# lachlanhurst/balance-robot-mujoco-rl

Measured on AMD Instinct MI355X. Metric: env-steps/sec, higher is better.
Workload: dtype f32; 1 GPU; Env03-v2, 65536 env instances per GPU (65536 total), random policy U(-1,1)^2, auto-reset on, 250 substeps of 2e-5 s per env step; envs_per_gpu=65536, substeps=250, parallelism=env-sharded x1, no collective, lane_grouping=True, streams=1, preroll_steps=300, preroll_stationary=True

## Files before the change

balance_robot_mujoco_rl_amd/csrc/brs_kernels.hip:

```cpp
#include <hip/hip_runtime.h>

#include <cstdio>
#include <cstdlib>
#include <cstring>
#include <string>
#include <vector>

#include "../../include/brs.h"
#if defined(BRS_TIMING)
__device__ unsigned long long brs_dbg[16];
__device__ unsigned long long brs_dbg_wave[4096];
#define BRS_TIMING_LANE_WORDS 153
#endif
#include "brs_state.hpp"

using namespace brs;

namespace {

template <bool BLK> constexpr int lane_words() { return BLK ? LDS_WORDS_ENV03 : LDS_WORDS_ENV01; }

template <bool BLK> __device__ __forceinline__ Store<float> lane_store(float* lds) {
  const int wave = threadIdx.x >> 6, lane = threadIdx.x & 63;
  return Store<float>{lds + wave * (64 * lane_words<BLK>()) + lane, 64};
}

template <int VARIANT> __device__ __forceinline__ Params<float> fold_params(const Params<float>& rt) {
  if constexpr (VARIANT < 0) return rt;
  else {
    constexpr Params<float> c = make_params<float>(VARIANT, 0u, -1, 0, 0, 0.0, 0, 0);
    Params<float> p = c;
    p.seed = rt.seed; p.gid_base = rt.gid_base; p.auto_reset = rt.auto_reset; p.noise = rt.noise;
    p.max_episode_steps = rt.max_episode_steps; p.nsub = rt.nsub;
    return p;
  }
}

constexpr int NBUCKET = 6;
__device__ __forceinline__ int bucket_of(int key, int e) {
  const int k = key & 3;
  if (k == 1) return 0;
  if (k == 2) return 4;
  if (k == 3) return 5;
  return (key & 4) ? ((e & 1) ? 3 : 1) : 2;
}
constexpr int GROUP_WORDS = 16;
template <bool BLK> __device__ __forceinline__ unsigned* group_counters(int* ii, int N) {
  return (unsigned*)(ii + ((size_t)Layout<BLK>::NI + 2) * N);
}

template <bool BLK, int VARIANT>
__device__ __forceinline__ void step_body(const Params<float>& Prt, const int N, double* __restrict__ d, float* __restrict__ f,
                                          int* __restrict__ ii, const float* __restrict__ actions, float* __restrict__ obs,
                                          float* __restrict__ reward, uint8_t* __restrict__ terminated,
                                          uint8_t* __restrict__ truncated, float* __restrict__ terminal_obs) {
  extern __shared__ float brs_lds_dyn[];
  float* lds = brs_lds_dyn;
  const int lane_slot = blockIdx.x * blockDim.x + threadIdx.x;
  if (lane_slot >= N) return;
  const Params<float> P = fold_params<VARIANT>(Prt);
#if defined(BRS_NO_PERM)
  const LaneIndex idx{nullptr, lane_slot};
#else
  const LaneIndex idx{BLK ? ii + (size_t)Layout<BLK>::NI * N : nullptr, lane_slot};
#endif
  Store<float> st = lane_store<BLK>(lds);
#if defined(BRS_TIMING) && defined(__HIP_DEVICE_COMPILE__)
  if ((threadIdx.x & 63) == 0) for (int k = 0; k < 16; k++) brs_tim_slots()[k] = 0;
#endif
  Stream<float> rng;
  float a0, a1;
  {
    const size_t i = idx.get();
    rng.open(P.seed, P.gid_base + (int64_t)i, 0u);
    a0 = actions[2 * i]; a1 = actions[2 * i + 1];
  }
  float o[6], to[6], rew;
  int te, tr, cls = 0;
  env_step_idx<float, BLK, float, LaneIndex>(P, st, rng, d, f, ii, (size_t)N, idx, a0, a1, o, to, rew, te, tr, BLK ? &cls : nullptr);
  const size_t i = idx.get();
  if constexpr (BLK) {
    ((uint8_t*)(ii + ((size_t)Layout<BLK>::NI + 1) * N))[i] = (uint8_t)cls;
    const int b = bucket_of(cls, (int)i);
    unsigned* cnt = group_counters<BLK>(ii, N);
#pragma unroll
    for (int k = 0; k < NBUCKET; k++) {
      const unsigned long long m = __ballot(b == k);
      if (m != 0ull && (threadIdx.x & 63) == (unsigned)(__ffsll((long long)m) - 1)) atomicAdd(&cnt[k], (unsigned)__popcll(m));
    }
  }
#if defined(BRS_TIMING) && defined(__HIP_DEVICE_COMPILE__)
  if ((threadIdx.x & 63) == 0) {
    for (int k = 0; k < 12; k++) atomicAdd(&brs_dbg[k], brs_tim_slots()[k]);
    atomicMax(&brs_dbg[12], brs_tim_slots()[8]);
    atomicMax(&brs_dbg[13], brs_tim_slots()[9]);
    unsigned hw, xcc;
    asm volatile("s_getreg_b32 %0, hwreg(HW_REG_HW_ID)" : "=s"(hw));
    asm volatile("s_getreg_b32 %0, hwreg(HW_REG_XCC_ID)" : "=s"(xcc));
    const unsigned w = (blockIdx.x * blockDim.x + threadIdx.x) >> 6;
    if (w < 1024) {
      brs_dbg_wave[4 * w + 0] = brs_tim_slots()[8]; brs_dbg_wave[4 * w + 1] = brs_tim_slots()[9];
      brs_dbg_wave[4 * w + 2] = hw; brs_dbg_wave[4 * w + 3] = xcc;
    }
  }
#endif
#pragma unroll
  for (int k = 0; k < 6; k++) obs[6 * (size_t)i + k] = o[k];
  if (terminal_obs) {
#pragma unroll
    for (int k = 0; k < 6; k++) terminal_obs[6 * (size_t)i + k] = to[k];
  }
  reward[i] = rew;
  terminated[i] = (uint8_t)te;
  truncated[i] = (uint8_t)tr;
}

#define BRS_STEP_ARGS                                                                                                      \
  const Params<float> Prt, const int N, double *__restrict__ d, float *__restrict__ f, int *__restrict__ ii,              \
      const float *__restrict__ actions, float *__restrict__ obs, float *__restrict__ reward, uint8_t *__restrict__ terminated, \
      uint8_t *__restrict__ truncated, float *__restrict__ terminal_obs
template <bool BLK, int VARIANT> __global__ void __launch_bounds__(256) brs_step_kernel(BRS_STEP_ARGS) {
  step_body<BLK, VARIANT>(Prt, N, d, f, ii, actions, obs, reward, terminated, truncated, terminal_obs);
}
template <int VARIANT> __global__ void __launch_bounds__(64, 2) brs_step_kernel_occ2(BRS_STEP_ARGS) {
  step_body<false, VARIANT>(Prt, N, d, f, ii, actions, obs, reward, terminated, truncated, terminal_obs);
}

template <bool BLK>
__global__ void __launch_bounds__(256) brs_reset_kernel(const Params<float> P, const int N, double* __restrict__ d,
                                                        float* __restrict__ f, int* __restrict__ ii,
                                                        const uint8_t* __restrict__ mask, float* __restrict__ obs) {
  const int i = blockIdx.x * blockDim.x + threadIdx.x;
  if (i >= N) return;
  if (mask && !mask[i]) return;
  EnvState<float, BLK> S;
  load_state<float, BLK>(S, d, f, ii, (size_t)N, (size_t)i);
  Stream<float> rng;
  rng.open(P.seed, P.gid_base + (int64_t)i, S.rng_ctr);
  float o[6];
  Sim<float, BLK>::env_reset(P, S, rng, o);
  S.rng_ctr = rng.ctr;
  store_state<float, BLK>(S, d, f, ii, (size_t)N, (size_t)i);
#pragma unroll
  for (int k = 0; k < 6; k++) obs[6 * (size_t)i + k] = o[k];
}

template <bool BLK>
__global__ void __launch_bounds__(256) brs_physics_kernel(const Params<float> P, const int N, double* __restrict__ d,
                                                          float* __restrict__ f, int* __restrict__ ii,
                                                          const float* __restrict__ ctrl, const int nsub) {
  extern __shared__ float brs_lds_dyn[];
  float* lds = brs_lds_dyn;
  const int i = blockIdx.x * blockDim.x + threadIdx.x;
  if (i >= N) return;
  Store<float> st = lane_store<BLK>(lds);
  physics_mem<float, BLK, float>(P, st, d, f, ii, (size_t)N, (size_t)i, ctrl[2 * (size_t)i], ctrl[2 * (size_t)i + 1], nsub);
}

constexpr int GROUP_THREADS = 256, GROUP_ENVS = 1024;
__global__ void __launch_bounds__(GROUP_THREADS) brs_group_kernel(const int N, const uint8_t* __restrict__ keys, int* __restrict__ perm,
                                                                  unsigned* __restrict__ ctr) {
  constexpr int NV = GROUP_ENVS / 64;
  __shared__ unsigned wcnt[NV][NBUCKET], woff[NBUCKET];
  const int lane = threadIdx.x & 63, w = threadIdx.x >> 6;
  int b[GROUP_ENVS / GROUP_THREADS];
  unsigned long long mine[GROUP_ENVS / GROUP_THREADS];
#pragma unroll
  for (int j = 0; j < GROUP_ENVS / GROUP_THREADS; j++) {
    const int e = blockIdx.x * GROUP_ENVS + j * GROUP_THREADS + threadIdx.x;
    b[j] = e < N ? bucket_of(keys[e], e) : -1;
    mine[j] = 0ull;
#pragma unroll
    for (int k = 0; k < NBUCKET; k++) {
      const unsigned long long m = __ballot(b[j] == k);
      if (lane == 0) wcnt[j * (GROUP_THREADS / 64) + w][k] = (unsigned)__popcll(m);
      mine[j] = b[j] == k ? m : mine[j];
    }
  }
  __syncthreads();
  if (threadIdx.x < NBUCKET) {
    const int k = threadIdx.x;
    unsigned base = 0, tot = 0;
    for (int j = 0; j < k; j++) base += ctr[j];
    for (int v = 0; v < NV; v++) { const unsigned c = wcnt[v][k]; wcnt[v][k] = tot; tot += c; }
    woff[k] = base + (tot ? atomicAdd(&ctr[NBUCKET + k], tot) : 0u);
  }
  __syncthreads();
#pragma unroll
  for (int j = 0; j < GROUP_ENVS / GROUP_THREADS; j++) {
    const int e = blockIdx.x * GROUP_ENVS + j * GROUP_THREADS + threadIdx.x;
    if (b[j] >= 0) perm[woff[b[j]] + wcnt[j * (GROUP_THREADS / 64) + w][b[j]] + (unsigned)__popcll(mine[j] & ((1ull << lane) - 1ull))] = e;
  }
  __syncthreads();
  if (threadIdx.x == 0) {
    __threadfence();
    if (atomicAdd(&ctr[2 * NBUCKET], 1u) == gridDim.x - 1) {
#pragma unroll
      for (int k = 0; k <= 2 * NBUCKET; k++) ctr[k] = 0u;
    }
  }
}

thread_local std::string g_create_error;

}

struct brs_handle {
  Params<float> P;
  int N = 0, device = 0, bt = 64;
  bool blk = false;
  double* d = nullptr;
  float* f = nullptr;
  int* ii = nullptr;
  size_t nd = 0, nf = 0, ni = 0;
  bool folded = false;
  bool occ2 = false;
  bool grouping = false;
  int* perm() const { return ii + ni; }
  uint8_t* keys() const { return (uint8_t*)(ii + ni + (size_t)N); }
  unsigned* counters() const { return (unsigned*)(ii + ni + 2 * (size_t)N); }
  std::string err;
};

namespace {

struct DeviceGuard {
  int prev = -1;
  bool ok = true;
  explicit DeviceGuard(int dev) {
    if (hipGetDevice(&prev) != hipSuccess) prev = -1;
    if (prev != dev) ok = hipSetDevice(dev) == hipSuccess;
  }
  ~DeviceGuard() {
    if (prev >= 0) (void)hipSetDevice(prev);
  }
};

int fail(brs_handle* h, int code, const std::string& msg) {
  if (h) h->err = msg; else g_create_error = msg;
  return code;
}
#define BRS_HIP_TRY(h, expr)                                                                              \
  do {                                                                                                    \
    hipError_t e_ = (expr);                                                                               \
    if (e_ != hipSuccess) return fail(h, BRS_ERR_HIP, std::string(#expr) + ": " + hipGetErrorString(e_)); \
  } while (0)

#if defined(BRS_TIMING)
size_t lds_bytes(const brs_handle* h) { return (size_t)h->bt * BRS_TIMING_LANE_WORDS * sizeof(float) + (size_t)(h->bt / 64) * 128; }
#else
size_t lds_bytes(const brs_handle* h) { return (size_t)h->bt * (h->blk ? LDS_WORDS_ENV03 : LDS_WORDS_ENV01) * sizeof(float); }
#endif
int grid_of(const brs_handle* h) { return (h->N + h->bt - 1) / h->bt; }

template <bool BLK> int upload_state(brs_handle* h, const std::vector<double>& d, const std::vector<float>& f, const std::vector<int>& ii) {
  BRS_HIP_TRY(h, hipMemcpy(h->d, d.data(), d.size() * sizeof(double), hipMemcpyHostToDevice));
  BRS_HIP_TRY(h, hipMemcpy(h->f, f.data(), f.size() * sizeof(float), hipMemcpyHostToDevice));
  BRS_HIP_TRY(h, hipMemcpy(h->ii, ii.data(), ii.size() * sizeof(int), hipMemcpyHostToDevice));
  return BRS_OK;
}
int download_state(brs_handle* h, std::vector<double>& d, std::vector<float>& f, std::vector<int>& ii) {
  d.resize(h->nd); f.resize(h->nf); ii.resize(h->ni);
  BRS_HIP_TRY(h, hipDeviceSynchronize());
  BRS_HIP_TRY(h, hipMemcpy(d.data(), h->d, h->nd * sizeof(double), hipMemcpyDeviceToHost));
  BRS_HIP_TRY(h, hipMemcpy(f.data(), h->f, h->nf * sizeof(float), hipMemcpyDeviceToHost));
  BRS_HIP_TRY(h, hipMemcpy(ii.data(), h->ii, h->ni * sizeof(int), hipMemcpyDeviceToHost));
  return BRS_OK;
}

}

extern "C" {

int brs_sizes(int32_t variant, int32_t* nq, int32_t* nv, int32_t* nobs, int32_t* nact) {
  if (variant < 0 || variant > 5) return BRS_ERR_ARG;
  bool blk = variant == 2 || variant == 3;
  if (nq) *nq = blk ? 16 : 9;
  if (nv) *nv = blk ? 14 : 8;
  if (nobs) *nobs = 6;
  if (nact) *nact = 2;
  return BRS_OK;
}

int brs_create(const brs_config* cfg, brs_handle** out) {
  if (!cfg || !out) return fail(nullptr, BRS_ERR_ARG, "brs_create: null argument");
  *out = nullptr;
  if (cfg->variant < 0 || cfg->variant > 5) return fail(nullptr, BRS_ERR_ARG, "brs_create: unknown variant");
  if (cfg->num_envs <= 0) return fail(nullptr, BRS_ERR_ARG, "brs_create: num_envs must be > 0");
  if ((cfg->flags & BRS_FLAG_NOISE_ON) && (cfg->flags & BRS_FLAG_NOISE_OFF))
    return fail(nullptr, BRS_ERR_ARG, "brs_create: NOISE_ON and NOISE_OFF are exclusive");
  int bt = cfg->block_threads > 0 ? cfg->block_threads : 64;
  if (bt % 64 != 0 || bt > 256) return fail(nullptr, BRS_ERR_ARG, "brs_create: block_threads must be 64, 128, 192 or 256");
  int ndev = 0;
  hipError_t e = hipGetDeviceCount(&ndev);
  if (e != hipSuccess || ndev <= 0)
    return fail(nullptr, BRS_ERR_HIP, std::string("brs_create: no HIP device (") + hipGetErrorString(e) + "); there is no CPU fallback");
  if (cfg->device < 0 || cfg->device >= ndev) return fail(nullptr, BRS_ERR_ARG, "brs_create: device ordinal out of range");
  brs_handle* h = new brs_handle();
  h->N = cfg->num_envs; h->device = cfg->device; h->bt = bt; h->blk = cfg->variant == 2 || cfg->variant == 3;
  int noise = (cfg->flags & BRS_FLAG_NOISE_ON) ? 1 : ((cfg->flags & BRS_FLAG_NOISE_OFF) ? 0 : -1);
  h->P = make_params<float>(cfg->variant, cfg->flags & BRS_FLAG_AUTO_RESET, noise, cfg->max_episode_steps, cfg->substeps,
                            cfg->timestep, cfg->seed, cfg->env_index_base);
  DeviceGuard g(h->device);
  size_t N = (size_t)h->N;
  if (h->blk) { h->nd = Layout<true>::ND * N; h->nf = Layout<true>::NF * N; h->ni = Layout<true>::NI * N; }
  else { h->nd = Layout<false>::ND * N; h->nf = Layout<false>::NF * N; h->ni = Layout<false>::NI * N; }
  auto bail = [&](const std::string& m) { std::string mm = m; brs_destroy(h); return fail(nullptr, BRS_ERR_HIP, mm); };
  if (!g.ok) return bail("brs_create: hipSetDevice failed");
  if (hipMalloc(&h->d, (h->nd + 7 * N) * sizeof(double)) != hipSuccess) return bail("brs_create: hipMalloc(fp64 state) failed");
  if (hipMalloc(&h->f, h->nf * sizeof(float)) != hipSuccess) return bail("brs_create: hipMalloc(fp32 state) failed");
  if (hipMalloc(&h->ii, (h->ni + 2 * N + GROUP_WORDS) * sizeof(int)) != hipSuccess) return bail("brs_create: hipMalloc(int state) failed");
  std::vector<double> d(h->nd);
  std::vector<float> f(h->nf);
  std::vector<int> ii(h->ni);
  int rc;
  if (h->blk) { hostconv::init_state<true>(d.data(), f.data(), ii.data(), N, cfg->seed, cfg->env_index_base); rc = upload_state<true>(h, d, f, ii); }
  else { hostconv::init_state<false>(d.data(), f.data(), ii.data(), N, cfg->seed, cfg->env_index_base); rc = upload_state<false>(h, d, f, ii); }
  if (rc != BRS_OK) return bail("brs_create: initial upload failed: " + h->err);
  {
    std::vector<int> id(2 * N, 0);
    for (size_t k = 0; k < N; k++) id[k] = (int)k;
    if (hipMemcpy(h->perm(), id.data(), 2 * N * sizeof(int), hipMemcpyHostToDevice) != hipSuccess) return bail("brs_create: lane map init failed");
    if (hipMemset(h->counters(), 0, GROUP_WORDS * sizeof(int)) != hipSuccess) return bail("brs_create: counter init failed");
    h->grouping = h->blk && !(cfg->flags & BRS_FLAG_NO_LANE_GROUPING);
    h->folded = !(cfg->timestep > 0 && cfg->timestep != 2e-5) && !std::getenv("BRS_NO_FOLD");
    h->occ2 = !h->blk && std::getenv("BRS_ENV01_OCC1") == nullptr;
  }
  size_t lb = lds_bytes(h);
  hipError_t ea = hipSuccess;
  auto want = [&](const void* fn) { if (ea == hipSuccess) ea = hipFuncSetAttribute(fn, hipFuncAttributeMaxDynamicSharedMemorySize, (int)lb); };
  if (h->blk) {
    want((const void*)brs_step_kernel<true, -1>); want((const void*)brs_step_kernel<true, ENV03_V1>);
    want((const void*)brs_step_kernel<true, ENV03_V2>); want((const void*)brs_physics_kernel<true>);
  } else {
    want((const void*)brs_step_kernel<false, -1>); want((const void*)brs_step_kernel<false, ENV01_V1>);
    want((const void*)brs_step_kernel<false, ENV01_V2>); want((const void*)brs_step_kernel<false, ENV01_V3>);
    want((const void*)brs_step_kernel<false, ENV02_V1>); want((const void*)brs_physics_kernel<false>);
    want((const void*)brs_step_kernel_occ2<-1>); want((const void*)brs_step_kernel_occ2<ENV01_V1>);
    want((const void*)brs_step_kernel_occ2<ENV01_V2>); want((const void*)brs_step_kernel_occ2<ENV01_V3>);
    want((const void*)brs_step_kernel_occ2<ENV02_V1>);
  }
  if (ea != hipSuccess) return bail(std::string("brs_create: hipFuncSetAttribute: ") + hipGetErrorString(ea));
  *out = h;
  return BRS_OK;
}

int brs_destroy(brs_handle* h) {
  if (!h) return BRS_ERR_STATE;
  {
    DeviceGuard g(h->device);
    if (h->d) (void)hipFree(h->d);
    if (h->f) (void)hipFree(h->f);
    if (h->ii) (void)hipFree(h->ii);
  }
  delete h;
  return BRS_OK;
}

const char* brs_last_error(const brs_handle* h) { return h ? h->err.c_str() : g_create_error.c_str(); }

int brs_reset(brs_handle* h, const uint8_t* mask_dev, float* obs_dev, void* stream) {
  if (!h) return BRS_ERR_STATE;
  if (!obs_dev) return fail(h, BRS_ERR_ARG, "brs_reset: obs_dev is null");
  DeviceGuard g(h->device);
  hipStream_t s = (hipStream_t)stream;
  if (h->blk) hipLaunchKernelGGL(brs_reset_kernel<true>, dim3(grid_of(h)), dim3(h->bt), 0, s, h->P, h->N, h->d, h->f, h->ii, mask_dev, obs_dev);
  else hipLaunchKernelGGL(brs_reset_kernel<false>, dim3(grid_of(h)), dim3(h->bt), 0, s, h->P, h->N, h->d, h->f, h->ii, mask_dev, obs_dev);
  BRS_HIP_TRY(h, hipGetLastError());
  return BRS_OK;
}

int brs_step(brs_handle* h, const float* actions_dev, float* obs_dev, float* reward_dev, uint8_t* terminated_dev,
             uint8_t* truncated_dev, float* terminal_obs_dev, void* stream) {
  if (!h) return BRS_ERR_STATE;
  if (!actions_dev || !obs_dev || !reward_dev || !terminated_dev || !truncated_dev)
    return fail(h, BRS_ERR_ARG, "brs_step: null buffer");
  DeviceGuard g(h->device);
  hipStream_t s = (hipStream_t)stream;
  size_t lb = lds_bytes(h);
  const dim3 grid(grid_of(h)), block(h->bt);
#define BRS_LAUNCH_STEP(BLK_, VAR_)                                                                                          \
  hipLaunchKernelGGL((brs_step_kernel<BLK_, VAR_>), grid, block, lb, s, h->P, h->N, h->d, h->f, h->ii, actions_dev, obs_dev, \
                     reward_dev, terminated_dev, truncated_dev, terminal_obs_dev)
#define BRS_LAUNCH_OCC2(VAR_)                                                                                              \
  hipLaunchKernelGGL((brs_step_kernel_occ2<VAR_>), grid, block, lb, s, h->P, h->N, h->d, h->f, h->ii, actions_dev, obs_dev, \
                     reward_dev, terminated_dev, truncated_dev, terminal_obs_dev)
  if (!h->blk && h->occ2 && h->bt == 64) {
    switch (h->folded ? h->P.variant : -1) {
      case ENV01_V1: BRS_LAUNCH_OCC2(ENV01_V1); break;
      case ENV01_V2: BRS_LAUNCH_OCC2(ENV01_V2); break;
      case ENV01_V3: BRS_LAUNCH_OCC2(ENV01_V3); break;
      case ENV02_V1: BRS_LAUNCH_OCC2(ENV02_V1); break;
      default: BRS_LAUNCH_OCC2(-1);
    }
  } else
  switch (h->folded ? h->P.variant : -1) {
    case ENV01_V1: BRS_LAUNCH_STEP(false, ENV01_V1); break;
    case ENV01_V2: BRS_LAUNCH_STEP(false, ENV01_V2); break;
    case ENV01_V3: BRS_LAUNCH_STEP(false, ENV01_V3); break;
    case ENV02_V1: BRS_LAUNCH_STEP(false, ENV02_V1); break;
    case ENV03_V1: BRS_LAUNCH_STEP(true, ENV03_V1); break;
    case ENV03_V2: BRS_LAUNCH_STEP(true, ENV03_V2); break;
    default:
      if (h->blk) BRS_LAUNCH_STEP(true, -1); else BRS_LAUNCH_STEP(false, -1);
  }
#undef BRS_LAUNCH_STEP
#undef BRS_LAUNCH_OCC2
  BRS_HIP_TRY(h, hipGetLastError());
  if (h->blk) {
    if (h->grouping) {
      hipLaunchKernelGGL(brs_group_kernel, dim3((h->N + GROUP_ENVS - 1) / GROUP_ENVS), dim3(GROUP_THREADS), 0, s, h->N, h->keys(), h->perm(), h->counters());
      BRS_HIP_TRY(h, hipGetLastError());
    } else
      BRS_HIP_TRY(h, hipMemsetAsync(h->counters(), 0, GROUP_WORDS * sizeof(int), s));
  }
  return BRS_OK;
}

int brs_physics(brs_handle* h, const float* ctrl_dev, int32_t nsub, void* stream) {
  if (!h) return BRS_ERR_STATE;
  if (!ctrl_dev || nsub < 0) return fail(h, BRS_ERR_ARG, "brs_physics: bad argument");
  DeviceGuard g(h->device);
  hipStream_t s = (hipStream_t)stream;
  size_t lb = lds_bytes(h);
  if (h->blk) hipLaunchKernelGGL(brs_physics_kernel<true>, dim3(grid_of(h)), dim3(h->bt), lb, s, h->P, h->N, h->d, h->f, h->ii, ctrl_dev, nsub);
  else hipLaunchKernelGGL(brs_physics_kernel<false>, dim3(grid_of(h)), dim3(h->bt), lb, s, h->P, h->N, h->d, h->f, h->ii, ctrl_dev, nsub);
  BRS_HIP_TRY(h, hipGetLastError());
  return BRS_OK;
}

#define BRS_STATE_ROUNDTRIP(h, MODIFY_T, MODIFY_F, WRITE)                                   \
  do {                                                                                     \
    if (!h) return BRS_ERR_STATE;                                                          \
    DeviceGuard g(h->device);                                                              \
    std::vector<double> d; std::vector<float> f; std::vector<int> ii;                      \
    int rc = download_state(h, d, f, ii);                                                  \
    if (rc != BRS_OK) return rc;                                                           \
    size_t N = (size_t)h->N; (void)N;                                                      \
    if (h->blk) { MODIFY_T; } else { MODIFY_F; }                                           \
    if (WRITE) { rc = h->blk ? upload_state<true>(h, d, f, ii) : upload_state<false>(h, d, f, ii); } \
    return rc;                                                                             \
  } while (0)

int brs_get_state(brs_handle* h, double* qpos, double* qvel, double* warm, double* time) {
  BRS_STATE_ROUNDTRIP(h, hostconv::get_state<true>(d.data(), f.data(), N, qpos, qvel, warm, time),
                      hostconv::get_state<false>(d.data(), f.data(), N, qpos, qvel, warm, time), false);
}
int brs_set_state(brs_handle* h, const double* qpos, const double* qvel, const double* warm, const double* time) {
  BRS_STATE_ROUNDTRIP(h, hostconv::set_state<true>(d.data(), f.data(), N, qpos, qvel, warm, time),
                      hostconv::set_state<false>(d.data(), f.data(), N, qpos, qvel, warm, time), true);
}
int brs_get_aux(brs_handle* h, double* aux) {
  if (!aux) return BRS_ERR_ARG;
  BRS_STATE_ROUNDTRIP(h, hostconv::get_aux<true>(d.data(), f.data(), ii.data(), N, aux),
                      hostconv::get_aux<false>(d.data(), f.data(), ii.data(), N, aux), false);
}
int brs_set_aux(brs_handle* h, const double* aux) {
  if (!aux) return BRS_ERR_ARG;
  BRS_STATE_ROUNDTRIP(h, hostconv::set_aux<true>(d.data(), f.data(), ii.data(), N, aux),
                      hostconv::set_aux<false>(d.data(), f.data(), ii.data(), N, aux), true);
}
int brs_get_xpose(brs_handle* h, double* xquat, double* xpos) {
  BRS_STATE_ROUNDTRIP(h, hostconv::get_xpose<true>(d.data(), N, xquat, xpos), hostconv::get_xpose<false>(d.data(), N, xquat, xpos), false);
}
int brs_set_xpose(brs_handle* h, const double* xquat, const double* xpos) {
  BRS_STATE_ROUNDTRIP(h, hostconv::set_xpose<true>(d.data(), N, xquat, xpos), hostconv::set_xpose<false>(d.data(), N, xquat, xpos), true);
}

int64_t brs_step_bytes_per_env(const brs_handle* h) {
  if (!h) return 0;
  size_t st = h->blk ? Layout<true>::bytes_per_env : Layout<false>::bytes_per_env;
  return (int64_t)(2 * st + 8 + 24 + 24 + 4 + 2);
}
#if defined(BRS_TIMING)
int brs_debug_waves(unsigned long long* out4096) {
  return hipMemcpyFromSymbol(out4096, HIP_SYMBOL(brs_dbg_wave), 4096 * sizeof(unsigned long long)) == hipSuccess ? BRS_OK : BRS_ERR_HIP;
}
int brs_debug_counters(unsigned long long* out16) {
  if (hipMemcpyFromSymbol(out16, HIP_SYMBOL(brs_dbg), 16 * sizeof(unsigned long long)) != hipSuccess) return BRS_ERR_HIP;
  unsigned long long z[16] = {0};
  if (hipMemcpyToSymbol(HIP_SYMBOL(brs_dbg), z, sizeof z) != hipSuccess) return BRS_ERR_HIP;
  return BRS_OK;
}
#endif
#ifndef BRS_BUILD_ID
#define BRS_BUILD_ID "unstamped"
#endif
const char* brs_build_id(void) { return BRS_BUILD_ID; }
const char* brs_step_kernel_name(const brs_handle* h) {
  if (!h) return "";
  static thread_local char name[64];
  const int var = h->folded ? h->P.variant : -1;
  if (!h->blk && h->occ2 && h->bt == 64) std::snprintf(name, sizeof name, "brs_step_kernel_occ2<%d>", var);
  else std::snprintf(name, sizeof name, "brs_step_kernel<%s, %d>", h->blk ? "true" : "false", var);
  return name;
}

}
```

balance_robot_mujoco_rl_amd/csrc/brs_state.hpp:

```cpp
#pragma once
#include <cmath>
#include <cstddef>
#include <cstdint>

#include "brs_core.hpp"

namespace brs {

template <bool BLK> struct Layout {
  static constexpr int NQ = BLK ? 16 : 9, NV = BLK ? 14 : 8;
  static constexpr int D_P = 0, D_Q = 3, D_TH = 7, D_TIME = 9, D_XQ = 10, D_XP = 14, D_BP = 17, D_BQ = 20, D_TIMER = 24;
  static constexpr int ND_POSE = BLK ? 25 : 17;
  static constexpr int D_V = ND_POSE, D_W = D_V + 3, D_WW = D_V + 6, D_BV = D_V + 8, D_BW = D_V + 11;
  static constexpr int ND = ND_POSE + (BRS_VEL64 ? NV : 0);
  static constexpr int F_V = 0, F_W = 3, F_WW = 6, F_A = 8, F_LASTPITCH = 8 + NV, F_EPRET = 9 + NV, F_BV = 10 + NV,
                       F_BW = 13 + NV;
  static constexpr int F_MUW = (BLK ? 16 : 10) + NV, F_DTS = F_MUW + 1, F_POFF = F_MUW + 2, F_TWS = F_MUW + 3;
  static constexpr int NF = F_MUW + 4;
  static constexpr int I_ELAPSED = 0, I_RNG = 1, I_SIDE = 2, I_BAD = 3, NI = 4;
  static constexpr size_t bytes_per_env = (size_t)ND * 8 + (size_t)NF * 4 + (size_t)NI * 4;
};

template <typename R, bool BLK, typename FT>
BRS_HD void load_state_phys(EnvState<R, BLK>& S, const double* d, const FT* f, const int* ii, size_t N, size_t i) {
  using L = Layout<BLK>;
#pragma unroll
  for (int k = 0; k < 3; k++) { S.p[k] = d[(L::D_P + k) * N + i]; S.xp[k] = d[(L::D_XP + k) * N + i]; }
#pragma unroll
  for (int k = 0; k < 4; k++) { S.q[k] = d[(L::D_Q + k) * N + i]; S.xq[k] = d[(L::D_XQ + k) * N + i]; }
  S.th[0] = d[(L::D_TH + 0) * N + i]; S.th[1] = d[(L::D_TH + 1) * N + i];
  S.time = d[L::D_TIME * N + i];
#pragma unroll
  for (int k = 0; k < 3; k++) { S.v[k] = (R)f[(L::F_V + k) * N + i]; S.w[k] = (R)f[(L::F_W + k) * N + i]; }
  S.ww[0] = (R)f[(L::F_WW + 0) * N + i]; S.ww[1] = (R)f[(L::F_WW + 1) * N + i];
#pragma unroll
  for (int k = 0; k < L::NV; k++) S.a[k] = (R)f[(L::F_A + k) * N + i];
  if constexpr (BLK) {
#pragma unroll
    for (int k = 0; k < 3; k++) {
      S.bp[k] = d[(L::D_BP + k) * N + i];
      S.bv[k] = (R)f[(L::F_BV + k) * N + i];
      S.bw[k] = (R)f[(L::F_BW + k) * N + i];
    }
#pragma unroll
    for (int k = 0; k < 4; k++) S.bq[k] = d[(L::D_BQ + k) * N + i];
  }
#if BRS_VEL64
#pragma unroll
  for (int k = 0; k < 3; k++) { S.vd[k] = d[(L::D_V + k) * N + i]; S.wd[k] = d[(L::D_W + k) * N + i]; S.v[k] = (R)S.vd[k]; S.w[k] = (R)S.wd[k]; }
  S.wwd[0] = d[(L::D_WW + 0) * N + i]; S.wwd[1] = d[(L::D_WW + 1) * N + i]; S.ww[0] = (R)S.wwd[0]; S.ww[1] = (R)S.wwd[1];
  if constexpr (BLK) {
#pragma unroll
    for (int k = 0; k < 3; k++) { S.bvd[k] = d[(L::D_BV + k) * N + i]; S.bwd[k] = d[(L::D_BW + k) * N + i]; S.bv[k] = (R)S.bvd[k]; S.bw[k] = (R)S.bwd[k]; }
  }
#endif
  S.rng_ctr = (uint32_t)ii[L::I_RNG * N + i];
  S.side_front = ii[L::I_SIDE * N + i];
  S.muw = (R)f[L::F_MUW * N + i];
  S.pnfr = 0; S.pnfb = 0; S.pnc = 0; S.psels = 0; S.pmR = 0; S.pmB = 0; S.pmC = 0;
}
template <typename R, bool BLK, typename FT>
BRS_HD void load_state_env(EnvState<R, BLK>& S, const double* d, const FT* f, const int* ii, size_t N, size_t i) {
  using L = Layout<BLK>;
  S.last_pitch = (R)f[L::F_LASTPITCH * N + i];
  S.ep_return = (R)f[L::F_EPRET * N + i];
  if constexpr (BLK) S.block_timer = d[L::D_TIMER * N + i]; else S.block_timer = -1.0;
  S.elapsed = ii[L::I_ELAPSED * N + i];
  S.bad = ii[L::I_BAD * N + i];
  S.dts = (R)f[L::F_DTS * N + i]; S.poff = (R)f[L::F_POFF * N + i]; S.tws = (R)f[L::F_TWS * N + i];
}
template <typename R, bool BLK, typename FT>
BRS_HD void load_state(EnvState<R, BLK>& S, const double* d, const FT* f, const int* ii, size_t N, size_t i) {
  load_state_phys<R, BLK, FT>(S, d, f, ii, N, i);
  load_state_env<R, BLK, FT>(S, d, f, ii, N, i);
}

template <typename R, bool BLK, typename FT>
BRS_HD void store_state(const EnvState<R, BLK>& S, double* d, FT* f, int* ii, size_t N, size_t i) {
  using L = Layout<BLK>;
#pragma unroll
  for (int k = 0; k < 3; k++) { d[(L::D_P + k) * N + i] = S.p[k]; d[(L::D_XP + k) * N + i] = S.xp[k]; }
#pragma unroll
  for (int k = 0; k < 4; k++) { d[(L::D_Q + k) * N + i] = S.q[k]; d[(L::D_XQ + k) * N + i] = S.xq[k]; }
  d[(L::D_TH + 0) * N + i] = S.th[0]; d[(L::D_TH + 1) * N + i] = S.th[1];
  d[L::D_TIME * N + i] = S.time;
#pragma unroll
  for (int k = 0; k < 3; k++) { f[(L::F_V + k) * N + i] = (FT)S.v[k]; f[(L::F_W + k) * N + i] = (FT)S.w[k]; }
  f[(L::F_WW + 0) * N + i] = (FT)S.ww[0]; f[(L::F_WW + 1) * N + i] = (FT)S.ww[1];
#pragma unroll
  for (int k = 0; k < L::NV; k++) f[(L::F_A + k) * N + i] = (FT)S.a[k];
  f[L::F_LASTPITCH * N + i] = (FT)S.last_pitch;
  f[L::F_EPRET * N + i] = (FT)S.ep_return;
  f[L::F_MUW * N + i] = (FT)S.muw; f[L::F_DTS * N + i] = (FT)S.dts; f[L::F_POFF * N + i] = (FT)S.poff; f[L::F_TWS * N + i] = (FT)S.tws;
  if constexpr (BLK) {
#pragma unroll
    for (int k = 0; k < 3; k++) {
      d[(L::D_BP + k) * N + i] = S.bp[k];
      f[(L::F_BV + k) * N + i] = (FT)S.bv[k];
      f[(L::F_BW + k) * N + i] = (FT)S.bw[k];
    }
#pragma unroll
    for (int k = 0; k < 4; k++) d[(L::D_BQ + k) * N + i] = S.bq[k];
    d[L::D_TIMER * N + i] = S.block_timer;
  }
#if BRS_VEL64
#pragma unroll
  for (int k = 0; k < 3; k++) { d[(L::D_V + k) * N + i] = S.vd[k]; d[(L::D_W + k) * N + i] = S.wd[k]; }
  d[(L::D_WW + 0) * N + i] = S.wwd[0]; d[(L::D_WW + 1) * N + i] = S.wwd[1];
  if constexpr (BLK) {
#pragma unroll
    for (int k = 0; k < 3; k++) { d[(L::D_BV + k) * N + i] = S.bvd[k]; d[(L::D_BW + k) * N + i] = S.bwd[k]; }
  }
#endif
  ii[L::I_ELAPSED * N + i] = S.elapsed;
  ii[L::I_RNG * N + i] = (int)S.rng_ctr;
  ii[L::I_SIDE * N + i] = S.side_front;
  ii[L::I_BAD * N + i] = S.bad;
}

template <typename R, bool BLK> BRS_HD int cost_class(const Params<R>& P, const EnvState<R, BLK>& S) {
  if constexpr (!BLK) return 0;
  else {
    const R T = (R)P.nsub * P.h, slack = (R)0.003;
    const R vb = sqrt_(S.bv[0] * S.bv[0] + S.bv[1] * S.bv[1] + S.bv[2] * S.bv[2]);
    const R vr = sqrt_(S.v[0] * S.v[0] + S.v[1] * S.v[1] + S.v[2] * S.v[2]) + (R)0.12 * sqrt_(S.w[0] * S.w[0] + S.w[1] * S.w[1] + S.w[2] * S.w[2]);
    const R reach = (vb + vr) * T + (R)0.5 * P.g * T * T + slack;
    int key = 0;
    const R low = (R)(S.bp[2] - P.floor_z_d) - P.block_brad - P.cc[CC_BLOCK_FLOOR].margin;
#if defined(BRS_CLASS_V1)
    key |= low < reach ? 1 : 0;
#else
    key |= low < max_(-S.bv[2], (R)0) * T + (R)0.5 * P.g * T * T + slack ? 1 : 0;
#endif
    R qf[4] = {(R)S.q[0], (R)S.q[1], (R)S.q[2], (R)S.q[3]}, RT[9];
    quat2mat_(qf, RT);
    const R d[3] = {(R)(S.bp[0] - S.p[0]), (R)(S.bp[1] - S.p[1]), (R)(S.bp[2] - S.p[2])};
    R dl[3];
    mulT_(RT, d, dl);
    const R rr = P.wheel_brad + P.block_brad + P.cc[CC_BLOCK_ROBOT].margin + reach;
    const R dz = dl[2] - P.wheel_pz, dxl = dl[0] + P.wheel_px, dxr = dl[0] - P.wheel_px;
    const R base = dl[1] * dl[1] + dz * dz;
    key |= (base + dxl * dxl < rr * rr || base + dxr * dxr < rr * rr) ? 2 : 0;
    const R dzt = dl[2] - P.torso_cz, rt = P.torso_brad + P.block_brad + P.cc[CC_BLOCK_ROBOT].margin + reach;
    key |= (dl[0] * dl[0] + dl[1] * dl[1] + dzt * dzt > rt * rt) ? 4 : 0;
    return key;
  }
}

struct FixedIndex {
  static constexpr bool SCRATCH = false;
  size_t i;
  BRS_HD size_t get() const { return i; }
  BRS_HD size_t slot_index() const { return i; }
};
struct LaneIndex {
  static constexpr bool SCRATCH = true;
  const volatile int* perm;
  int slot;
  BRS_HD size_t get() const { return perm ? (size_t)perm[slot] : (size_t)slot; }
  BRS_HD size_t slot_index() const { return (size_t)slot; }
};

template <typename R, bool BLK, typename FT, typename IDX>
BRS_HD void env_step_idx(const Params<R>& P, Store<R>& st, Stream<R>& rng, double* d, FT* f, int* ii, size_t N, const IDX& idx,
                         float a0, float a1, float* obs, float* terminal_obs, float& reward, int& terminated, int& truncated,
                         int* next_cost_class = nullptr) {
  using L = Layout<BLK>;
  using SimT = Sim<R, BLK>;
  EnvState<R, BLK> S;
  CtrlT<R> ctrlL, ctrlR;
  R rew;
  {
    const size_t i = idx.get();
    load_state_phys<R, BLK, FT>(S, d, f, ii, N, i);
    load_state_env<R, BLK, FT>(S, d, f, ii, N, i);
    rng.ctr = S.rng_ctr;
    rew = SimT::env_pre(P, S, rng, a0, a1, ctrlL, ctrlR);
    if (P.v3) f[L::F_TWS * N + i] = (FT)S.tws;
  }
  {
    typename SimT::SubCtx C;
    int k = 0;
    bool fresh = true;
    while (k < P.nsub) {
      BRS_TIC(8);
      if (fresh) {
        if (k == P.nsub - 1) {
          const size_t sl = idx.slot_index();
          constexpr int FQ = IDX::SCRATCH ? L::ND : L::D_XQ, FP = IDX::SCRATCH ? L::ND + 4 : L::D_XP;
#pragma unroll
          for (int j = 0; j < 4; j++) d[(FQ + j) * N + sl] = S.q[j];
#pragma unroll
          for (int j = 0; j < 3; j++) d[(FP + j) * N + sl] = S.p[j];
        }
        SimT::sub_begin(P, st, S, ctrlL, ctrlR, C);
        fresh = false;
      }
      if (!C.conv) SimT::sub_iter(P, st, S, C);
      if (C.conv) {
        SimT::sub_end(P, S, C);
        k++;
        fresh = true;
      }
      BRS_TOC(8);
#if defined(BRS_TIMING) && defined(__HIP_DEVICE_COMPILE__)
      if (BRS_LEADER()) brs_tim_slots()[9] += 1ull;
#endif
    }
  }
  S.derive_vel32();
#if defined(__HIP_DEVICE_COMPILE__)
  asm volatile("" ::: "memory");
#endif
  const size_t i = idx.get();
  rng.gid = P.gid_base + (int64_t)i;
  if (P.nsub > 0) {
    const size_t sl = idx.slot_index();
    constexpr int FQ = IDX::SCRATCH ? L::ND : L::D_XQ, FP = IDX::SCRATCH ? L::ND + 4 : L::D_XP;
#pragma unroll
    for (int j = 0; j < 4; j++) S.xq[j] = d[(FQ + j) * N + sl];
#pragma unroll
    for (int j = 0; j < 3; j++) S.xp[j] = d[(FP + j) * N + sl];
  }
  load_state_env<R, BLK, FT>(S, d, f, ii, N, i);
  SimT::env_post(P, S, rng, rew, obs, terminal_obs, reward, terminated, truncated);
  S.rng_ctr = rng.ctr;
  if (next_cost_class) *next_cost_class = cost_class<R, BLK>(P, S);
  store_state<R, BLK, FT>(S, d, f, ii, N, i);
}
template <typename R, bool BLK, typename FT>
BRS_HD void env_step_mem(const Params<R>& P, Store<R>& st, Stream<R>& rng, double* d, FT* f, int* ii, size_t N, size_t i,
                         float a0, float a1, float* obs, float* terminal_obs, float& reward, int& terminated, int& truncated,
                         int* next_cost_class = nullptr) {
  env_step_idx<R, BLK, FT, FixedIndex>(P, st, rng, d, f, ii, N, FixedIndex{i}, a0, a1, obs, terminal_obs, reward, terminated, truncated,
                                       next_cost_class);
}

template <typename R, bool BLK, typename FT>
BRS_HD void physics_mem(const Params<R>& P, Store<R>& st, double* d, FT* f, int* ii, size_t N, size_t i, CtrlT<R> ctrlL, CtrlT<R> ctrlR, int nsub) {
  using SimT = Sim<R, BLK>;
  EnvState<R, BLK> S;
  load_state<R, BLK, FT>(S, d, f, ii, N, i);
  typename SimT::SubCtx C;
  int k = 0;
  bool fresh = true;
  while (k < nsub) {
    if (fresh) {
#pragma unroll
      for (int j = 0; j < 4; j++) S.xq[j] = S.q[j];
#pragma unroll
      for (int j = 0; j < 3; j++) S.xp[j] = S.p[j];
      SimT::sub_begin(P, st, S, ctrlL, ctrlR, C);
      fresh = false;
    }
    if (!C.conv) SimT::sub_iter(P, st, S, C);
    if (C.conv) {
      SimT::sub_end(P, S, C);
      k++;
      fresh = true;
    }
  }
  S.derive_vel32();
  store_state<R, BLK, FT>(S, d, f, ii, N, i);
}

namespace hostconv {

inline bool isnan_bits(double x) { union { double f; uint64_t u; } c; c.f = x; return (c.u & 0x7fffffffffffffffull) > 0x7ff0000000000000ull; }
inline void quat_norm(double* q) {
  double n = std::sqrt(q[0] * q[0] + q[1] * q[1] + q[2] * q[2] + q[3] * q[3]);
  if (n < 1e-15) { q[0] = 1; q[1] = q[2] = q[3] = 0; return; }
  for (int k = 0; k < 4; k++) q[k] /= n;
}
inline void quat_mat(const double* q, double* M) { quat2mat_<double>(q, M); }

template <bool BLK, typename FT>
inline void init_state(double* d, FT* f, int* ii, size_t N, uint64_t seed, int64_t gid_base) {
  using L = Layout<BLK>;
  for (size_t k = 0; k < (size_t)L::ND * N; k++) d[k] = 0;
  for (size_t k = 0; k < (size_t)L::NF * N; k++) f[k] = 0;
  for (size_t k = 0; k < (size_t)L::NI * N; k++) ii[k] = 0;
  for (size_t i = 0; i < N; i++) {
    d[(L::D_Q + 0) * N + i] = 1; d[(L::D_XQ + 0) * N + i] = 1;
    f[L::F_MUW * N + i] = (FT)1;
    if (BLK) { d[(L::D_BQ + 0) * N + i] = 1; d[L::D_TIMER * N + i] = -1.0; }
    uint32_t o[4];
    int64_t gid = gid_base + (int64_t)i;
    philox4x32_10(0u, 0u, (uint32_t)((uint64_t)gid & 0xffffffffu), (uint32_t)((uint64_t)gid >> 32),
                  (uint32_t)(seed & 0xffffffffu), (uint32_t)(seed >> 32), o);
    double u0 = (double)(o[0] >> 8) * (1.0 / 16777216.0);
    ii[L::I_SIDE * N + i] = u0 > 0.5 ? 1 : 0;
    ii[L::I_RNG * N + i] = 1;
  }
}

template <bool BLK, typename FT>
inline void set_state(double* d, FT* f, size_t N, const double* qpos, const double* qvel, const double* warm,
                      const double* time) {
  using L = Layout<BLK>;
  for (size_t i = 0; i < N; i++) {
    if (qpos) {
      const double* q = qpos + i * L::NQ;
      double qt[4] = {q[3], q[4], q[5], q[6]};
      quat_norm(qt);
      for (int k = 0; k < 3; k++) { d[(L::D_P + k) * N + i] = q[k]; d[(L::D_XP + k) * N + i] = q[k]; }
      for (int k = 0; k < 4; k++) { d[(L::D_Q + k) * N + i] = qt[k]; d[(L::D_XQ + k) * N + i] = qt[k]; }
      d[(L::D_TH + 0) * N + i] = q[7]; d[(L::D_TH + 1) * N + i] = q[8];
      if (BLK) {
        double qb[4] = {q[12], q[13], q[14], q[15]};
        quat_norm(qb);
        for (int k = 0; k < 3; k++) d[(L::D_BP + k) * N + i] = q[9 + k];
        for (int k = 0; k < 4; k++) d[(L::D_BQ + k) * N + i] = qb[k];
      }
    }
    if (qvel) {
      const double* v = qvel + i * L::NV;
      for (int k = 0; k < 3; k++) { f[(L::F_V + k) * N + i] = (FT)v[k]; f[(L::F_W + k) * N + i] = (FT)v[3 + k]; }
      f[(L::F_WW + 0) * N + i] = (FT)v[6]; f[(L::F_WW + 1) * N + i] = (FT)v[7];
      if (BLK)
        for (int k = 0; k < 3; k++) { f[(L::F_BV + k) * N + i] = (FT)v[8 + k]; f[(L::F_BW + k) * N + i] = (FT)v[11 + k]; }
#if BRS_VEL64
      for (int k = 0; k < L::NV; k++) d[(L::D_V + k) * N + i] = v[k];
#endif
    }
    if (warm) {
      const double* a = warm + i * L::NV;
      double qt[4], M[9];
      for (int k = 0; k < 4; k++) qt[k] = d[(L::D_Q + k) * N + i];
      quat_mat(qt, M);
      for (int k = 0; k < 3; k++) f[(L::F_A + k) * N + i] = (FT)(M[k] * a[0] + M[3 + k] * a[1] + M[6 + k] * a[2]);
      for (int k = 3; k < 8; k++) f[(L::F_A + k) * N + i] = (FT)a[k];
      if (BLK) {
        for (int k = 0; k < 4; k++) qt[k] = d[(L::D_BQ + k) * N + i];
        quat_mat(qt, M);
        for (int k = 0; k < 3; k++) f[(L::F_A + 8 + k) * N + i] = (FT)(M[k] * a[8] + M[3 + k] * a[9] + M[6 + k] * a[10]);
        for (int k = 11; k < 14; k++) f[(L::F_A + k) * N + i] = (FT)a[k];
      }
    }
    if (time) d[L::D_TIME * N + i] = time[i];
  }
}

template <bool BLK, typename FT>
inline void get_state(const double* d, const FT* f, size_t N, double* qpos, double* qvel, double* warm, double* time) {
  using L = Layout<BLK>;
  for (size_t i = 0; i < N; i++) {
    if (qpos) {
      double* q = qpos + i * L::NQ;
      for (int k = 0; k < 3; k++) q[k] = d[(L::D_P + k) * N + i];
      for (int k = 0; k < 4; k++) q[3 + k] = d[(L::D_Q + k) * N + i];
      q[7] = d[(L::D_TH + 0) * N + i]; q[8] = d[(L::D_TH + 1) * N + i];
      if (BLK) {
        for (int k = 0; k < 3; k++) q[9 + k] = d[(L::D_BP + k) * N + i];
        for (int k = 0; k < 4; k++) q[12 + k] = d[(L::D_BQ + k) * N + i];
      }
    }
    if (qvel) {
      double* v = qvel + i * L::NV;
      for (int k = 0; k < 3; k++) { v[k] = f[(L::F_V + k) * N + i]; v[3 + k] = f[(L::F_W + k) * N + i]; }
      v[6] = f[(L::F_WW + 0) * N + i]; v[7] = f[(L::F_WW + 1) * N + i];
      if (BLK)
        for (int k = 0; k < 3; k++) { v[8 + k] = f[(L::F_BV + k) * N + i]; v[11 + k] = f[(L::F_BW + k) * N + i]; }
#if BRS_VEL64
      for (int k = 0; k < L::NV; k++) v[k] = d[(L::D_V + k) * N + i];
#endif
    }
    if (warm) {
      double* a = warm + i * L::NV;
      double qt[4], M[9], ab[3];
      for (int k = 0; k < 4; k++) qt[k] = d[(L::D_XQ + k) * N + i];
      quat_mat(qt, M);
      for (int k = 0; k < 3; k++) ab[k] = f[(L::F_A + k) * N + i];
      for (int k = 0; k < 3; k++) a[k] = M[3 * k] * ab[0] + M[3 * k + 1] * ab[1] + M[3 * k + 2] * ab[2];
      for (int k = 3; k < 8; k++) a[k] = f[(L::F_A + k) * N + i];
      if (BLK) {
        for (int k = 0; k < 4; k++) qt[k] = d[(L::D_BQ + k) * N + i];
        quat_mat(qt, M);
        for (int k = 0; k < 3; k++) ab[k] = f[(L::F_A + 8 + k) * N + i];
        for (int k = 0; k < 3; k++) a[8 + k] = M[3 * k] * ab[0] + M[3 * k + 1] * ab[1] + M[3 * k + 2] * ab[2];
        for (int k = 11; k < 14; k++) a[k] = f[(L::F_A + k) * N + i];
      }
    }
    if (time) time[i] = d[L::D_TIME * N + i];
  }
}

template <bool BLK, typename FT> inline void get_aux(const double* d, const FT* f, const int* ii, size_t N, double* aux) {
  using L = Layout<BLK>;
  for (size_t i = 0; i < N; i++) {
    double* a = aux + 14 * i;
    a[0] = f[L::F_LASTPITCH * N + i];
    double t = BLK ? d[L::D_TIMER * N + i] : -1.0;
    { union { double f; uint64_t u; } qn; qn.u = 0x7ff8000000000000ull; a[1] = t < 0 ? qn.f : t; }
    a[2] = ii[L::I_ELAPSED * N + i]; a[3] = (uint32_t)ii[L::I_RNG * N + i]; a[4] = ii[L::I_SIDE * N + i];
    double xq[4];
    for (int k = 0; k < 4; k++) xq[k] = d[(L::D_XQ + k) * N + i];
    double p, y;
    Sim<double, BLK>::pitch_yaw(xq, p, y);
    a[5] = p; a[6] = f[L::F_EPRET * N + i]; a[7] = ii[L::I_BAD * N + i]; a[8] = a[9] = 0;
    a[10] = f[L::F_MUW * N + i]; a[11] = f[L::F_DTS * N + i]; a[12] = f[L::F_POFF * N + i]; a[13] = f[L::F_TWS * N + i];
  }
}
template <bool BLK, typename FT> inline void set_aux(double* d, FT* f, int* ii, size_t N, const double* aux) {
  using L = Layout<BLK>;
  for (size_t i = 0; i < N; i++) {
    const double* a = aux + 14 * i;
    f[L::F_LASTPITCH * N + i] = (FT)a[0];
    if (BLK) d[L::D_TIMER * N + i] = isnan_bits(a[1]) ? -1.0 : a[1];
    ii[L::I_ELAPSED * N + i] = (int)a[2]; ii[L::I_RNG * N + i] = (int)(uint32_t)a[3]; ii[L::I_SIDE * N + i] = a[4] != 0;
    f[L::F_EPRET * N + i] = (FT)a[6];
    f[L::F_MUW * N + i] = (FT)a[10]; f[L::F_DTS * N + i] = (FT)a[11]; f[L::F_POFF * N + i] = (FT)a[12]; f[L::F_TWS * N + i] = (FT)a[13];
  }
}
template <bool BLK> inline void get_xpose(const double* d, size_t N, double* xq, double* xp) {
  using L = Layout<BLK>;
  for (size_t i = 0; i < N; i++) {
    if (xq) for (int k = 0; k < 4; k++) xq[4 * i + k] = d[(L::D_XQ + k) * N + i];
    if (xp) for (int k = 0; k < 3; k++) xp[3 * i + k] = d[(L::D_XP + k) * N + i];
  }
}
template <bool BLK> inline void set_xpose(double* d, size_t N, const double* xq, const double* xp) {
  using L = Layout<BLK>;
  for (size_t i = 0; i < N; i++) {
    if (xq) for (int k = 0; k < 4; k++) d[(L::D_XQ + k) * N + i] = xq[4 * i + k];
    if (xp) for (int k = 0; k < 3; k++) d[(L::D_XP + k) * N + i] = xp[3 * i + k];
  }
}

}
}
```

Baseline: 13.56 million env-steps/s.

## Pack rare collision classes into capped lanes per wave with far-env padding

Replaces the six-bucket grouping with an eight-bucket lane plan driven by the raw class key. Buckets whose key carries the 0x2 bit are spread across waves with at most a capped number of lanes each, and the remaining lanes are filled with cheap far-away environments, so that expensive contact work is divided over more waves instead of piling onto a few. The cap applies only when the number of waves is small relative to the CU count. It also extends the timing/debug per-wave dump. The risk is extra permutation arithmetic and more divergent mixing inside waves.

```diff
diff --git a/balance_robot_mujoco_rl_amd/csrc/brs_kernels.hip b/balance_robot_mujoco_rl_amd/csrc/brs_kernels.hip
--- a/balance_robot_mujoco_rl_amd/csrc/brs_kernels.hip
+++ b/balance_robot_mujoco_rl_amd/csrc/brs_kernels.hip
@@ -9,7 +9,7 @@
 #include "../../include/brs.h"
 #if defined(BRS_TIMING)
 __device__ unsigned long long brs_dbg[16];
-__device__ unsigned long long brs_dbg_wave[4096];
+__device__ unsigned long long brs_dbg_wave[16 * 1024];
 #define BRS_TIMING_LANE_WORDS 153
 #endif
 #include "brs_state.hpp"
@@ -36,15 +36,9 @@
   }
 }
 
-constexpr int NBUCKET = 6;
-__device__ __forceinline__ int bucket_of(int key, int e) {
-  const int k = key & 3;
-  if (k == 1) return 0;
-  if (k == 2) return 4;
-  if (k == 3) return 5;
-  return (key & 4) ? ((e & 1) ? 3 : 1) : 2;
-}
-constexpr int GROUP_WORDS = 16;
+constexpr int NBUCKET = LM_NBUCKET;
+constexpr int GROUP_WORDS = 32;
+static_assert(2 * NBUCKET + 1 <= GROUP_WORDS, "bucket counters do not fit");
 template <bool BLK> __device__ __forceinline__ unsigned* group_counters(int* ii, int N) {
   return (unsigned*)(ii + ((size_t)Layout<BLK>::NI + 2) * N);
 }
@@ -67,6 +61,12 @@
   Store<float> st = lane_store<BLK>(lds);
 #if defined(BRS_TIMING) && defined(__HIP_DEVICE_COMPILE__)
   if ((threadIdx.x & 63) == 0) for (int k = 0; k < 16; k++) brs_tim_slots()[k] = 0;
+  if constexpr (BLK) {
+    const int key = ((const uint8_t*)(ii + ((size_t)Layout<BLK>::NI + 1) * N))[idx.get()];
+    unsigned long long ck = 0ull;
+    for (int k = 0; k < 8; k++) ck |= (unsigned long long)__popcll(__ballot(key == k)) << (8 * k);
+    if ((threadIdx.x & 63) == 0) { brs_tim_slots()[14] = ck; brs_tim_slots()[15] = ck; }
+  }
 #endif
   Stream<float> rng;
   float a0, a1;
@@ -81,7 +81,7 @@
   const size_t i = idx.get();
   if constexpr (BLK) {
     ((uint8_t*)(ii + ((size_t)Layout<BLK>::NI + 1) * N))[i] = (uint8_t)cls;
-    const int b = bucket_of(cls, (int)i);
+    const int b = cls;
     unsigned* cnt = group_counters<BLK>(ii, N);
 #pragma unroll
     for (int k = 0; k < NBUCKET; k++) {
@@ -99,8 +99,9 @@
     asm volatile("s_getreg_b32 %0, hwreg(HW_REG_XCC_ID)" : "=s"(xcc));
     const unsigned w = (blockIdx.x * blockDim.x + threadIdx.x) >> 6;
     if (w < 1024) {
-      brs_dbg_wave[4 * w + 0] = brs_tim_slots()[8]; brs_dbg_wave[4 * w + 1] = brs_tim_slots()[9];
-      brs_dbg_wave[4 * w + 2] = hw; brs_dbg_wave[4 * w + 3] = xcc;
+      for (int k = 0; k < 12; k++) brs_dbg_wave[16 * w + k] = brs_tim_slots()[k];
+      brs_dbg_wave[16 * w + 12] = hw; brs_dbg_wave[16 * w + 13] = xcc;
+      brs_dbg_wave[16 * w + 14] = BLK ? brs_tim_slots()[14] : 0ull; brs_dbg_wave[16 * w + 15] = BLK ? brs_tim_slots()[15] : 0ull;
     }
   }
 #endif
@@ -159,16 +160,17 @@
 
 constexpr int GROUP_THREADS = 256, GROUP_ENVS = 1024;
 __global__ void __launch_bounds__(GROUP_THREADS) brs_group_kernel(const int N, const uint8_t* __restrict__ keys, int* __restrict__ perm,
-                                                                  unsigned* __restrict__ ctr) {
+                                                                  unsigned* __restrict__ ctr, const unsigned cap) {
   constexpr int NV = GROUP_ENVS / 64;
-  __shared__ unsigned wcnt[NV][NBUCKET], woff[NBUCKET];
+  __shared__ unsigned wcnt[NV][NBUCKET], woff[NBUCKET], cnt[NBUCKET];
+  __shared__ LanePlan plan;
   const int lane = threadIdx.x & 63, w = threadIdx.x >> 6;
   int b[GROUP_ENVS / GROUP_THREADS];
   unsigned long long mine[GROUP_ENVS / GROUP_THREADS];
 #pragma unroll
   for (int j = 0; j < GROUP_ENVS / GROUP_THREADS; j++) {
     const int e = blockIdx.x * GROUP_ENVS + j * GROUP_THREADS + threadIdx.x;
-    b[j] = e < N ? bucket_of(keys[e], e) : -1;
+    b[j] = e < N ? (int)keys[e] : -1;
     mine[j] = 0ull;
 #pragma unroll
     for (int k = 0; k < NBUCKET; k++) {
@@ -180,16 +182,21 @@
   __syncthreads();
   if (threadIdx.x < NBUCKET) {
     const int k = threadIdx.x;
-    unsigned base = 0, tot = 0;
-    for (int j = 0; j < k; j++) base += ctr[j];
+    unsigned tot = 0;
+    cnt[k] = ctr[k];
     for (int v = 0; v < NV; v++) { const unsigned c = wcnt[v][k]; wcnt[v][k] = tot; tot += c; }
-    woff[k] = base + (tot ? atomicAdd(&ctr[NBUCKET + k], tot) : 0u);
-  }
+    woff[k] = tot ? atomicAdd(&ctr[NBUCKET + k], tot) : 0u;
+  }
+  __syncthreads();
+  if (threadIdx.x == 0) plan = lane_plan(cnt, cap);
   __syncthreads();
 #pragma unroll
   for (int j = 0; j < GROUP_ENVS / GROUP_THREADS; j++) {
     const int e = blockIdx.x * GROUP_ENVS + j * GROUP_THREADS + threadIdx.x;
-    if (b[j] >= 0) perm[woff[b[j]] + wcnt[j * (GROUP_THREADS / 64) + w][b[j]] + (unsigned)__popcll(mine[j] & ((1ull << lane) - 1ull))] = e;
+    if (b[j] >= 0) {
+      const unsigned r = woff[b[j]] + wcnt[j * (GROUP_THREADS / 64) + w][b[j]] + (unsigned)__popcll(mine[j] & ((1ull << lane) - 1ull));
+      perm[lane_slot(plan, cnt, b[j], r)] = e;
+    }
   }
   __syncthreads();
   if (threadIdx.x == 0) {
@@ -216,6 +223,7 @@
   bool folded = false;
   bool occ2 = false;
   bool grouping = false;
+  unsigned wheel_cap = LM_WAVE;
   int* perm() const { return ii + ni; }
   uint8_t* keys() const { return (uint8_t*)(ii + ni + (size_t)N); }
   unsigned* counters() const { return (unsigned*)(ii + ni + 2 * (size_t)N); }
@@ -323,6 +331,9 @@
     if (hipMemcpy(h->perm(), id.data(), 2 * N * sizeof(int), hipMemcpyHostToDevice) != hipSuccess) return bail("brs_create: lane map init failed");
     if (hipMemset(h->counters(), 0, GROUP_WORDS * sizeof(int)) != hipSuccess) return bail("brs_create: counter init failed");
     h->grouping = h->blk && !(cfg->flags & BRS_FLAG_NO_LANE_GROUPING);
+    int cus = 0;
+    if (hipDeviceGetAttribute(&cus, hipDeviceAttributeMultiprocessorCount, h->device) != hipSuccess) return bail("brs_create: CU count query failed");
+    h->wheel_cap = (N + LM_WAVE - 1) / LM_WAVE <= 4 * (size_t)cus ? (unsigned)LM_RARE_CAP : (unsigned)LM_WAVE;
     h->folded = !(cfg->timestep > 0 && cfg->timestep != 2e-5) && !std::getenv("BRS_NO_FOLD");
     h->occ2 = !h->blk && std::getenv("BRS_ENV01_OCC1") == nullptr;
   }
@@ -409,7 +420,7 @@
   BRS_HIP_TRY(h, hipGetLastError());
   if (h->blk) {
     if (h->grouping) {
-      hipLaunchKernelGGL(brs_group_kernel, dim3((h->N + GROUP_ENVS - 1) / GROUP_ENVS), dim3(GROUP_THREADS), 0, s, h->N, h->keys(), h->perm(), h->counters());
+      hipLaunchKernelGGL(brs_group_kernel, dim3((h->N + GROUP_ENVS - 1) / GROUP_ENVS), dim3(GROUP_THREADS), 0, s, h->N, h->keys(), h->perm(), h->counters(), h->wheel_cap);
       BRS_HIP_TRY(h, hipGetLastError());
     } else
       BRS_HIP_TRY(h, hipMemsetAsync(h->counters(), 0, GROUP_WORDS * sizeof(int), s));
@@ -473,8 +484,8 @@
   return (int64_t)(2 * st + 8 + 24 + 24 + 4 + 2);
 }
 #if defined(BRS_TIMING)
-int brs_debug_waves(unsigned long long* out4096) {
-  return hipMemcpyFromSymbol(out4096, HIP_SYMBOL(brs_dbg_wave), 4096 * sizeof(unsigned long long)) == hipSuccess ? BRS_OK : BRS_ERR_HIP;
+int brs_debug_waves(unsigned long long* out16384) {
+  return hipMemcpyFromSymbol(out16384, HIP_SYMBOL(brs_dbg_wave), 16 * 1024 * sizeof(unsigned long long)) == hipSuccess ? BRS_OK : BRS_ERR_HIP;
 }
 int brs_debug_counters(unsigned long long* out16) {
   if (hipMemcpyFromSymbol(out16, HIP_SYMBOL(brs_dbg), 16 * sizeof(unsigned long long)) != hipSuccess) return BRS_ERR_HIP;
diff --git a/balance_robot_mujoco_rl_amd/csrc/brs_state.hpp b/balance_robot_mujoco_rl_amd/csrc/brs_state.hpp
--- a/balance_robot_mujoco_rl_amd/csrc/brs_state.hpp
+++ b/balance_robot_mujoco_rl_amd/csrc/brs_state.hpp
@@ -145,6 +145,68 @@
     key |= (dl[0] * dl[0] + dl[1] * dl[1] + dzt * dzt > rt * rt) ? 4 : 0;
     return key;
   }
+}
+
+#ifndef BRS_RARE_CAP
+#define BRS_RARE_CAP 16
+#endif
+enum { LM_NBUCKET = 8, LM_PLAIN = 0, LM_FAR = 4, LM_WAVE = 64, LM_RARE_CAP = BRS_RARE_CAP };
+static_assert(LM_RARE_CAP >= 1 && LM_RARE_CAP <= LM_WAVE, "BRS_RARE_CAP: 1..64 lanes per wave");
+BRS_HD constexpr int lm_bucket_at(int o) {
+  return o == 0 ? 3 : o == 1 ? 2 : o == 2 ? 7 : o == 3 ? 6 : o == 4 ? LM_PLAIN : o == 5 ? 1 : 5;
+}
+struct LanePlan {
+  unsigned pos[LM_NBUCKET];
+  unsigned per[LM_NBUCKET];
+  unsigned nfar[LM_NBUCKET];
+  unsigned far0[LM_NBUCKET];
+  unsigned rest_pos, rest_far0;
+};
+BRS_HD LanePlan lane_plan(const unsigned* cnt, unsigned cap = LM_RARE_CAP) {
+  LanePlan L;
+  unsigned pos = 0, far_left = cnt[LM_FAR], far_used = 0;
+#pragma unroll
+  for (int o = 0; o < LM_NBUCKET - 1; o++) {
+    const int k = lm_bucket_at(o);
+    const unsigned c = cnt[k];
+    unsigned per = (k & 2) ? cap : (unsigned)LM_WAVE;
+    unsigned need = 0;
+    if (c > 0) {
+      if (per < LM_WAVE) {
+        const unsigned nw = min_((c + per - 1) / per, (c + far_left) / LM_WAVE);
+        if (pos % LM_WAVE != 0 || nw <= (c - 1) / LM_WAVE) per = LM_WAVE;
+        else per = (c + nw - 1) / nw;
+        need = (c + per - 1) / per * LM_WAVE - c;
+      }
+      if (per == LM_WAVE) {
+        need = (LM_WAVE - (pos + c) % LM_WAVE) % LM_WAVE;
+        if (need > far_left) need = 0;
+      }
+    }
+    L.pos[k] = pos; L.per[k] = per; L.nfar[k] = need; L.far0[k] = far_used;
+    pos += c + need; far_used += need; far_left -= need;
+  }
+  L.pos[LM_FAR] = 0; L.per[LM_FAR] = LM_WAVE; L.nfar[LM_FAR] = 0; L.far0[LM_FAR] = 0;
+  L.rest_pos = pos; L.rest_far0 = far_used;
+  return L;
+}
+BRS_HD unsigned lane_slot(const LanePlan& L, const unsigned* cnt, int b, unsigned r) {
+  if (b != LM_FAR) {
+    const unsigned per = L.per[b];
+    return per == LM_WAVE ? L.pos[b] + r : L.pos[b] + LM_WAVE * (r / per) + r % per;
+  }
+#pragma unroll
+  for (int k = 0; k < LM_NBUCKET; k++) {
+    if (k == LM_FAR || r - L.far0[k] >= L.nfar[k]) continue;
+    const unsigned j = r - L.far0[k], per = L.per[k], c = cnt[k];
+    if (per == LM_WAVE) return L.pos[k] + c + j;
+    const unsigned f = LM_WAVE - per, nw = (c + per - 1) / per, full = (nw - 1) * f;
+    return j < full ? L.pos[k] + LM_WAVE * (j / f) + per + j % f : L.pos[k] + LM_WAVE * (nw - 1) + (c - (nw - 1) * per) + (j - full);
+  }
+  return L.rest_pos + (r - L.rest_far0);
+}
+BRS_HD unsigned lane_slot(int b, unsigned r, const unsigned* cnt, unsigned cap = LM_RARE_CAP) {
+  return lane_slot(lane_plan(cnt, cap), cnt, b, r);
 }
 
 struct FixedIndex {
```

Result: faster. 14.95 million env-steps/s (median of 6 runs) (+10.2%).
